# spcl/EBCC

Measured on AMD Instinct MI355X. Metric: fp32 GB/s encode+decode, 721x1440 ERA5 frames MAX_ERROR=0.5, higher is better.
Workload: dtype f32; 1 GPU; 256-frame batch 721x1440 fp32 per GPU, base_cr=30 MAX_ERROR=0.5 (BASELINE configs[1]); frames_per_gpu=256, parallelism=frames sharded over 1 GPU(s), no collective, hw_queues=4, encode_slices=3

## Files before the change

ebcc_amd/csrc/j2k.hip:

```cpp
#include <algorithm>
#include <cstring>
#include <vector>

#include "../../include/ebcc_hip.h"
#include "engine.hpp"
#include "j2k.hpp"

namespace ebcc {

bool j2k_create(ebcc_hip_ctx *ctx)
{
    J2kBuffers *jb = new J2kBuffers();
    ctx->j2k = jb;
    const int period = ctx->tile_period;
    std::vector<std::vector<J2kBlock>> tile_blocks((size_t) period);
    int stride = 0;
    for (int k = 0; k < period; k++) {
        jb->geoms.push_back(make_j2k_geom(ctx->height, ctx->width, tile_blocks[(size_t) k], k * ctx->height));
        stride = std::max(stride, jb->geoms.back().nblocks);
    }
    for (J2kGeom &t : jb->geoms) { t.period = period; t.stride = stride; }
    jb->geom = jb->geoms[0];
    const J2kGeom &g = jb->geom;
    const size_t n_pix = ctx->n_pix, F = ctx->max_frames;
    const size_t total = F * (size_t) stride, groups = (total + 63) / 64;
    jb->max_frames = (int) F;
    jb->fs = ctx->rb.fs;
    jb->stream_cap = ((n_pix * 3 + 4096 + 63) / 64) * 64;
    bool ok = true;
    ok &= (jb->d_geom = (J2kGeom *) ctx_alloc<uint8_t>(ctx, sizeof(J2kGeom) * (size_t) period)) != nullptr;
    ok &= (jb->d_blocks = (J2kBlock *) ctx_alloc<uint8_t>(ctx, sizeof(J2kBlock) * (size_t) period * (size_t) stride)) != nullptr;
    ok &= (jb->d_blkmap = ctx_alloc<uint16_t>(ctx, (size_t) period * n_pix)) != nullptr;
    ok &= (jb->B = ctx_alloc<float>(ctx, F * n_pix)) != nullptr;
    ok &= (jb->B2 = ctx_alloc<float>(ctx, F * n_pix)) != nullptr;
    ok &= (jb->Q6 = ctx_alloc<int32_t>(ctx, F * n_pix)) != nullptr;
    ok &= (jb->DEC = ctx_alloc<float>(ctx, F * n_pix)) != nullptr;
    ok &= (jb->V = ctx_alloc<int32_t>(ctx, F * n_pix)) != nullptr;
    ok &= (jb->BP = ctx_alloc<unsigned long long>(ctx, groups * kJ2kMaxPlanes * 64 * 64)) != nullptr;
    ok &= (jb->SGN = ctx_alloc<unsigned long long>(ctx, groups * 64 * 64)) != nullptr;
    ok &= (jb->SUF = ctx_alloc<unsigned long long>(ctx, groups * (kJ2kMaxPlanes + 2) * 64 * 64)) != nullptr;
    ok &= (jb->SPS = ctx_alloc<unsigned long long>(ctx, groups * 64 * 64)) != nullptr;
    ok &= (jb->VISP = ctx_alloc<unsigned long long>(ctx, groups * kJ2kMaxPlanes * 64 * 64)) != nullptr;
    ok &= (jb->ckpt = ctx_alloc<uint8_t>(ctx, groups * 64 * j2k_ckpt_block_bytes())) != nullptr;
    jb->SYM = nullptr;
    {
        const char *e = getenv("EBCC_T1_TWO_PHASE");
        jb->sym_rows = kJ2kSymRows;
        if (const char *r = getenv("EBCC_HIP_SYM_ROWS")) jb->sym_rows = std::max(1, std::min(kJ2kSymRows, atoi(r)));
        if (!e || atoi(e)) ok &= (jb->SYM = ctx_alloc<uint8_t>(ctx, groups * (size_t) ((jb->sym_rows + 1) & ~1) * 1024 + 256)) != nullptr;
    }
    ok &= (jb->seglen = ctx_alloc<uint16_t>(ctx, groups * (size_t) kJ2kSegCount * 64)) != nullptr;
    ok &= (jb->lanerows = ctx_alloc<uint32_t>(ctx, groups * 64)) != nullptr;
    ok &= (jb->qplane = (int *) ctx_alloc<int32_t>(ctx, groups * 64)) != nullptr;
    ok &= (jb->lastnp = (int *) ctx_alloc<int32_t>(ctx, groups * 64)) != nullptr;
    ok &= (jb->T1S = ctx_alloc<unsigned long long>(ctx, groups * kT1StateWords * 64)) != nullptr;
    ok &= (jb->blkmax = (int *) ctx_alloc<int32_t>(ctx, groups * 64)) != nullptr;
    ok &= (jb->numbps = (int *) ctx_alloc<int32_t>(ctx, groups * 64)) != nullptr;
    ok &= (jb->totalpasses = (int *) ctx_alloc<int32_t>(ctx, groups * 64)) != nullptr;
    ok &= (jb->cblk_len = (int *) ctx_alloc<int32_t>(ctx, groups * 64)) != nullptr;
    ok &= (jb->npass = (int *) ctx_alloc<int32_t>(ctx, groups * 64)) != nullptr;
    ok &= (jb->cand_cr = ctx_alloc<float>(ctx, F * 2)) != nullptr;
    ok &= (jb->cand_out = (int *) ctx_alloc<int32_t>(ctx, F * 6)) != nullptr;
    ok &= (jb->cand_npass = (int *) ctx_alloc<int32_t>(ctx, 2 * F * (size_t) stride)) != nullptr;
    ok &= (jb->cand_sel = (int *) ctx_alloc<int32_t>(ctx, F)) != nullptr;
    ok &= (jb->have_rate = (int *) ctx_alloc<int32_t>(ctx, F)) != nullptr;
    ok &= (jb->rate_path = (int *) ctx_alloc<int32_t>(ctx, F * 1536 * 3)) != nullptr;
    ok &= (jb->rate_path_n = (int *) ctx_alloc<int32_t>(ctx, 2 * F)) != nullptr;
    {
        int nodes = 0;
        for (const J2kGeom &t : jb->geoms) nodes = std::max(nodes, t.tree_nodes);
        J2kBuffers::RateCache &rc = jb->rate_cache;
        rc.nodes_cap = (nodes + 3) & ~3;
        rc.cap = stride * kJ2kMaxPasses;
        rc.ok = jb->rate_path_n ? jb->rate_path_n + F : nullptr;
        ok &= (rc.mnmx = ctx_alloc<double>(ctx, F * 2)) != nullptr;
        ok &= (rc.mval = (short *) ctx_alloc<uint16_t>(ctx, F * (size_t) rc.nodes_cap)) != nullptr;
        ok &= (rc.off = (int *) ctx_alloc<int32_t>(ctx, F * (size_t) (stride + 1))) != nullptr;
        ok &= (rc.crate = ctx_alloc<uint16_t>(ctx, F * (size_t) rc.cap)) != nullptr;
        ok &= (rc.cdisto = ctx_alloc<double>(ctx, F * (size_t) rc.cap)) != nullptr;
    }
    ok &= (jb->rates = (int *) ctx_alloc<int32_t>(ctx, groups * 64 * kJ2kMaxPasses)) != nullptr;
    ok &= (jb->disto = ctx_alloc<double>(ctx, groups * 64 * kJ2kMaxPasses)) != nullptr;
    ok &= (jb->cblk_bytes = ctx_alloc<uint8_t>(ctx, groups * 64 * kJ2kCblkBytes)) != nullptr;
    ok &= (jb->stream = ctx_alloc<uint8_t>(ctx, F * jb->stream_cap)) != nullptr;
    ok &= (jb->dec_table = (int *) ctx_alloc<int32_t>(ctx, groups * 64 * 4)) != nullptr;
    ok &= (jb->dec_order = (int *) ctx_alloc<int32_t>(ctx, groups * 64 + 128)) != nullptr;
    ok &= (jb->mq_order = (int *) ctx_alloc<int32_t>(ctx, groups * 64 + 256)) != nullptr;
    ok &= (jb->jf = (J2kFrame *) ctx_alloc<uint8_t>(ctx, sizeof(J2kFrame) * F)) != nullptr;
    ok &= (jb->partial = ctx_alloc<double>(ctx, F * kPartials)) != nullptr;
    ok &= (jb->partial_u = ctx_alloc<unsigned long long>(ctx, F * kPartials)) != nullptr;
    if (!ok) return false;
    poison_alloc(jb->cblk_bytes, groups * 64 * kJ2kCblkBytes);
    poison_alloc(jb->stream, F * jb->stream_cap);
    if (stride >= 65535) { set_error("too many code-blocks"); return false; }
    std::vector<uint16_t> map((size_t) period * n_pix, 0);
    std::vector<J2kBlock> blocks((size_t) period * (size_t) stride, J2kBlock{});
    for (int k = 0; k < period; k++) {
        const std::vector<J2kBlock> &tb = tile_blocks[(size_t) k];
        std::copy(tb.begin(), tb.end(), blocks.begin() + (size_t) k * (size_t) stride);
        for (size_t b = 0; b < tb.size(); b++)
            for (int y = 0; y < tb[b].h; y++)
                for (int x = 0; x < tb[b].w; x++) map[(size_t) k * n_pix + (size_t) (tb[b].y + y) * g.W + tb[b].x + x] = (uint16_t) b;
    }
    hipStream_t s = ctx->stream;
    EBCC_HIP_CHECK(hipMemcpyAsync(jb->d_geom, jb->geoms.data(), sizeof(J2kGeom) * (size_t) period, hipMemcpyHostToDevice, s));
    EBCC_HIP_CHECK(hipMemcpyAsync(jb->d_blocks, blocks.data(), sizeof(J2kBlock) * blocks.size(), hipMemcpyHostToDevice, s));
    EBCC_HIP_CHECK(hipMemcpyAsync(jb->d_blkmap, map.data(), map.size() * sizeof(uint16_t), hipMemcpyHostToDevice, s));
    EBCC_HIP_CHECK(hipHostMalloc(&ctx->h_jf, sizeof(J2kFrame) * F));
    EBCC_HIP_CHECK(hipHostMalloc((void **) &ctx->h_table, sizeof(int) * 4 * total));
    EBCC_HIP_CHECK(hipMemsetAsync(jb->jf, 0, sizeof(J2kFrame) * F, s));
    EBCC_HIP_CHECK(hipMemsetAsync(jb->rate_path_n, 0, sizeof(int) * 2 * F, s));
    wait_stream(s);
    return true;
}

void j2k_destroy(ebcc_hip_ctx *ctx)
{
    delete static_cast<J2kBuffers *>(ctx->j2k);
    ctx->j2k = nullptr;
    if (ctx->stream2) { hipStreamSynchronize(ctx->stream2); hipStreamDestroy(ctx->stream2); ctx->stream2 = nullptr; }
}

namespace {

struct BitReader {
    const uint8_t *p, *end;
    unsigned buf = 0;
    int ct = 0;
    int bit()
    {
        if (ct == 0) {
            buf = (buf << 8) & 0xFFFF;
            ct = buf == 0xFF00 ? 7 : 8;
            if (p < end) buf |= *p++;
        }
        ct--;
        return (buf >> ct) & 1;
    }
    int bits(int n) { int v = 0; for (int i = n - 1; i >= 0; i--) v |= bit() << i; return v; }
    void align() { if ((buf & 0xFF) == 0xFF && p < end) p++; ct = 0; }
};

struct HostTree {
    const J2kBand *bd;
    std::vector<int> val, low;
    explicit HostTree(const J2kBand &b) : bd(&b)
    {
        int n = 0;
        for (int l = 0; l < b.tree_levels; l++) n += b.lvl_w[l] * b.lvl_h[l];
        val.assign(n, 999); low.assign(n, 0);
    }
    bool decode(BitReader &br, int cx, int cy, int threshold)
    {
        int lowv = 0, idx = 0;
        for (int l = bd->tree_levels - 1; l >= 0; l--) {
            idx = bd->lvl_off[l] + (cy >> l) * bd->lvl_w[l] + (cx >> l);
            if (lowv > low[idx]) low[idx] = lowv; else lowv = low[idx];
            while (lowv < threshold && lowv < val[idx]) {
                if (br.bit()) val[idx] = lowv; else ++lowv;
            }
            low[idx] = lowv;
        }
        return val[idx] < threshold;
    }
// ... 440 lines not shown
```

ebcc_amd/csrc/j2k.hpp:

```cpp
#pragma once

#include <vector>

#include "../../include/ebcc_hip.h"
#include "common.hpp"
#include "residual.hpp"

namespace ebcc {

constexpr int kJ2kRes = 6;
constexpr int kJ2kBands = 3 * kJ2kRes - 2;
constexpr int kJ2kMaxPlanes = 26;
constexpr int kJ2kMaxPasses = 3 * kJ2kMaxPlanes;
constexpr int kJ2kCblkBytes = 16 * 1024;
constexpr int kT1StateWords = 66 + 4 * 64;

struct J2kBand {
    int res, orient, level;
    int x0, y0, x1, y1;
    int offx, offy;
    int ncw, nch;
    int first_block;
    int expn, mant, numbps;
    float step_enc, step_dec;
// ... 35 lines not shown
constexpr int kJ2kSegCount = kJ2kMaxPlanes * 3 * 16;
constexpr int kJ2kSymRows = (4096 * (kJ2kMaxPlanes + 2)) / 16 + kJ2kSegCount;
constexpr int kJ2kCkptPerBlock = kJ2kMaxPasses * 16;

constexpr int kJ2kCkptWords = 8;
__host__ __device__ inline size_t j2k_ckpt_block_bytes() { return (size_t) kJ2kCkptWords * kJ2kCkptPerBlock * 4; }
struct J2kCkptView {
    std::uint32_t *rec;
    __host__ __device__ std::uint32_t *slot(std::uint32_t i) const { return rec + i * kJ2kCkptWords; }
    __host__ __device__ static J2kCkptView of(void *all, size_t gid)
    {
        return J2kCkptView{(std::uint32_t *) ((unsigned char *) all + gid * j2k_ckpt_block_bytes())};
    }
};

struct J2kFrame {
    float cr;
    float target;
    int maxlen;
    int body_bytes;
    int stream_bytes;
    unsigned long long nbad;
    double err_sum;
    int overflow;
    int keep;
    float hdr_share;
    unsigned int bad_limit;
    unsigned int bad_seen;
};

struct J2kBuffers {
    J2kGeom geom;
    std::vector<J2kGeom> geoms;
    J2kGeom *d_geom;
    J2kBlock *d_blocks;
    std::uint16_t *d_blkmap;
    int max_frames;
    float *B;
    float *B2;
    int32_t *Q6;
    float *DEC;
    unsigned long long *BP;
    unsigned long long *SGN;
    unsigned long long *SUF;
    unsigned long long *SPS;
    unsigned long long *VISP;
    void *ckpt;
    uint8_t *SYM;
    int sym_rows;
    std::uint16_t *seglen;
    std::uint32_t *lanerows;
    int *qplane;
    int *lastnp;
    unsigned long long *T1S;
    int *blkmax;
    int *numbps;
    int *totalpasses;
    int *cblk_len;
    int *rates;
    double *disto;
    int *npass;
    float *cand_cr;
    int *cand_out;
    int *cand_npass;
    int *cand_sel;
    int *have_rate;
    int *rate_path;
    int *rate_path_n;
    struct RateCache {
        int *ok;
        double *mnmx;
        short *mval;
        int *off;
        unsigned short *crate;
        double *cdisto;
        int nodes_cap, cap;
    } rate_cache;
    uint8_t *cblk_bytes;
    uint8_t *stream;
    size_t stream_cap;
    int32_t *V;
    int *dec_table;
    int *dec_order;
    int *mq_order;
    J2kFrame *jf;
    FrameState *fs;
    double *partial;
    unsigned long long *partial_u;
};

enum T1Kernel { T1_ENCODE = 0, T1_MQ = 1, T1_RESUME = 2, T1_DECODE = 3 };
int t1_lanes_per_wave(int kernel, int total_blocks = 0);

J2kGeom make_j2k_geom(int H, int W, std::vector<J2kBlock> &blocks, int ty0 = 0);

struct J2kWindow {
    int row0, col0, rows, cols;
    int rx0[kJ2kRes], rx1[kJ2kRes], ry0[kJ2kRes], ry1[kJ2kRes];
    int band[kJ2kBands][4];
};
bool j2k_window_plan(const J2kGeom &g, size_t row0, size_t col0, size_t rows, size_t cols, J2kWindow &w);
bool j2k_window_supported(const J2kGeom &g);
bool j2k_window_keeps(const J2kGeom &g, const J2kBlock &b, const J2kWindow &w, int rect[4]);
constexpr int kL5Pairs = 60;
struct J2kStripRange { int strip0, strips, pos0, pos1, pieces; };
inline J2kStripRange j2k_cone_span(const J2kWindow &w, int r)
{
    const int strip0 = (w.rx0[r] / 2) / kL5Pairs;
    return J2kStripRange{strip0, ((w.rx1[r] - 1) / 2) / kL5Pairs - strip0 + 1, w.ry0[r] / 2, (w.ry1[r] - 1) / 2 + 1, 1};
}
int j2k_first_fused(const J2kBuffers &jb);
struct J2kBoxEntry {
    int frame, slot, row0, col0;
    int strip0[kJ2kRes], strips[kJ2kRes], pos0[kJ2kRes], pos1[kJ2kRes];
    int pad[4];
};
struct J2kPlacement {
    int rows, cols;
    unsigned long long at, pitch;
};
struct J2kBoxList {
    J2kBoxEntry *h_table, *table;
    J2kPlacement *h_place, *place;
    size_t n;
    int rows, cols;
};
struct J2kRegion {
    enum Kind { Frames, Window, List } kind = Frames;
    J2kWindow cone{};
    J2kBoxList list{};
    float *out = nullptr;
};
bool j2k_list_check(const char *who, const J2kGeom &g, size_t n_frames, const ebcc_hip_placed_box *boxes, size_t n_boxes, size_t out_floats,
                    uint8_t *keep = nullptr, J2kBoxEntry *table = nullptr, J2kPlacement *place = nullptr, int first_fused = kJ2kRes,
                    int *max_rows = nullptr, int *max_cols = nullptr);
bool j2k_boxes_as_placed(const char *who, const ebcc_hip_box *boxes, size_t n_boxes, size_t rows, size_t cols,
                         std::vector<ebcc_hip_placed_box> &placed, size_t *out_floats);
int j2k_selfcheck_div65535();

void launch_input_stats(const float *data, int n_frames, size_t n_pix, FrameState *fs, hipStream_t s);
void launch_j2k_analysis(const float *data, const J2kBuffers &jb, int n_frames, hipStream_t s);
void launch_j2k_tier1(const J2kBuffers &jb, int n_frames, hipStream_t s, bool single_kernel);
bool j2k_tier1_retry(const J2kBuffers &jb, int n_frames, const J2kFrame *host_jf, hipStream_t s);
// ... 14 lines not shown
```

ebcc_amd/csrc/j2k_rate.hip:

```cpp
#include <cfloat>
#include <cmath>
#include <cstdlib>
#include <mutex>

#include "j2k.hpp"
#include "t1_core.hpp"
#include "t1_device.hpp"

namespace ebcc {

int j2k_inverse_dwt(float *B, const int32_t *V, const float *data, const J2kBuffers &jb, int n_frames, const FrameState *fs,
                    const int *active, hipStream_t s, int keep_field, const J2kWindow *win = nullptr, float *win_out = nullptr);

namespace {

constexpr int kMainHeaderBytes = 135;
constexpr int kRateTrieNodes = 1536;
#ifndef EBCC_RATE_THREADS
#define EBCC_RATE_THREADS 512
#endif
constexpr int kRateThreads = EBCC_RATE_THREADS;
constexpr int kWriteThreads = 256;

__device__ inline int floorlog2d(int a) { return a > 1 ? 31 - __clz(a) : 0; }
// ... 876 lines not shown
        int running = 0;
        for (int base_b = 0; base_b < g.nblocks; base_b += kWriteThreads) {
            const int b = base_b + lane;
            int v = 0;
            if (b < g.nblocks && L.npass[b]) v = rates[(size_t) (gid0 + b) * kJ2kMaxPasses + L.npass[b] - 1];
            int x = v;
            for (int d = 1; d < 64; d <<= 1) { const int y = __shfl_up(x, d); if ((lane & 63) >= d) x += y; }
            if ((lane & 63) == 63) s_wave[lane >> 6] = x;
            __syncthreads();
            int before = running, tot = 0;
            for (int w = 0; w < kWriteThreads / 64; w++) { if (w < (lane >> 6)) before += s_wave[w]; tot += s_wave[w]; }
            if (b < g.nblocks) L.leafbits[b] = before + x - v;
            running += tot;
            __syncthreads();
        }
    }
    {
        const int wave = lane >> 6, wl = lane & 63;
        for (int blk = wave; blk < g.nblocks; blk += kWriteThreads / 64) {
            const int n = L.npass[blk];
            if (!n) continue;
            int bi = 0;
            while (bi + 1 < g.nbands && g.bands[bi + 1].first_block <= blk) bi++;
            const int res = g.bands[bi].res;
            const int seglen = rates[(size_t) (gid0 + blk) * kJ2kMaxPasses + n - 1];
            const uint8_t *src = cblk_bytes + (size_t) (gid0 + blk) * kJ2kCblkBytes;
            uint8_t *dst = base + s_off[res] + s_hdr[res] + (L.leafbits[blk] - L.leafbits[g.res_first[res]]);
            for (int i = wl; i < seglen; i += 64) dst[i] = src[i];
        }
    }
    if (lane == 0) {
        uint8_t *p = base;
        put16(p, 0xFF4F);
        put16(p, 0xFF51); put16(p, 41); put16(p, 0);
        put32(p, g.W); put32(p, g.H); put32(p, 0); put32(p, 0); put32(p, g.W); put32(p, g.H); put32(p, 0); put32(p, 0);
        put16(p, 1); *p++ = 15; *p++ = 1; *p++ = 1;
        put16(p, 0xFF52); put16(p, 12); *p++ = 0; *p++ = 0; put16(p, 1); *p++ = 0; *p++ = kJ2kRes - 1; *p++ = 4; *p++ = 4; *p++ = 0; *p++ = 0;
        put16(p, 0xFF5C); put16(p, 3 + 2 * kJ2kBands); *p++ = (uint8_t) (2 + (2 << 5));
        for (int bi = 0; bi < kJ2kBands; bi++) put16(p, (unsigned) ((g.bands[bi].expn << 11) | g.bands[bi].mant));
        const char com[] = "Created by OpenJPEG version 2.4.0";
        put16(p, 0xFF64); put16(p, 4 + 33); put16(p, 1);
        for (int i = 0; i < 33; i++) *p++ = (uint8_t) com[i];
        const int body = s_off[kJ2kRes] - (kMainHeaderBytes + 14);
        put16(p, 0xFF90); put16(p, 10); put16(p, 0); put32(p, (unsigned) (12 + 2 + body)); *p++ = 0; *p++ = 1;
        put16(p, 0xFF93);
        uint8_t *e = base + s_off[kJ2kRes];
        put16(e, 0xFFD9);
        jf[frame].stream_bytes = s_off[kJ2kRes] + 2;
        jf[frame].body_bytes = body;
    }
}

__global__ void k_finish_reduce(const double *partial, const unsigned long long *partial_u, J2kFrame *jf, int n, int n_partials,
                                const FrameState *fs, const int *active)
{
    int f = blockIdx.x * blockDim.x + threadIdx.x;
    if (f >= n || (active && !active[f]) || fs[f].const_field) return;
    jf[f].bad_seen = 0;
    double s = 0;
    unsigned long long b = 0;
    for (int i = 0; i < n_partials; i++) { s += partial[(size_t) f * kPartials + i]; b += partial_u[(size_t) f * kPartials + i]; }
    jf[f].err_sum = s;
    jf[f].nbad = b;
}


struct LdsTable {
    const __attribute__((address_space(3))) uint32_t *t;
    __device__ uint32_t operator()(int i) const { return t[i]; }
};
#define EBCC_LDS_MQ_TABLE(name)                                                              \
    __shared__ uint32_t name##_store[48];                                                    \
    if (threadIdx.x < 47) name##_store[threadIdx.x] = t1::mq_entry((int) threadIdx.x);       \
    __syncthreads();                                                                         \
    LdsTable name{(const __attribute__((address_space(3))) uint32_t *) name##_store}

__device__ __attribute__((aligned(16))) uint8_t g_ctx_tables[LdsCtx::kBytes];
void ensure_ctx_tables()
{
    static std::once_flag once[64];
    int dev = 0;
    EBCC_HIP_CHECK(hipGetDevice(&dev));
    std::call_once(once[dev & 63], [] {
        uint8_t t[LdsCtx::kBytes];
        make_ctx_tables(t);
        EBCC_HIP_CHECK(hipMemcpyToSymbol(HIP_SYMBOL(g_ctx_tables), t, sizeof t));
    });
}

struct DecStore {
    unsigned char *st;
    uint32_t lane8;
    int32_t *v;
    int W;
    __device__ unsigned long long &at(int row) const { return *(unsigned long long *) (st + ((uint32_t) row * 512u + lane8)); }
    __device__ unsigned long long &S(int y) { return at(y + 1); }
    __device__ unsigned long long &NEG(int y) { return at(66 + y); }
    __device__ unsigned long long &VIS(int y) { return at(130 + y); }
    __device__ unsigned long long &REF(int y) { return at(194 + y); }
    __device__ void set_sig(int x, int y, int neg, int plane)
    {
        int one = 1 << (plane + 1), val = one | (one >> 1);
        v[y * W + x] = neg ? -val : val;
    }
    __device__ void refine(int x, int y, int bit, int plane, int neg)
    {
        const int half = 1 << plane;
        atomicAdd(&v[y * W + x], (bit ^ neg) ? half : -half);
    }
// ... 147 lines not shown
    EBCC_LDS_MQ_TABLE(tab);
    const LdsCtx ctxp{(uint32_t) (uintptr_t) (__attribute__((address_space(3))) uint8_t *) ctx_store, 0u};
    int w = (int) blockIdx.x, slot0 = 0, lanes = tiers.lanes[3], end = total;
    {
        int t = 0;
        for (; t < 3; t++) {
            const int waves = tiers.n[t] / tiers.lanes[t];
            if (w < waves) { lanes = tiers.lanes[t]; end = slot0 + tiers.n[t]; break; }
            w -= waves; slot0 += tiers.n[t];
        }
    }
    if ((int) threadIdx.x >= lanes) return;
    const int slot = slot0 + w * lanes + (int) threadIdx.x;
    if (slot >= end || slot >= total) return;
    const int gid = order[slot];
    const int nb = geom->stride;
    const int frame = gid / nb, bi = gid - frame * nb;
    if (fs[frame].const_field) return;
    blocks = j2k_frame_blocks(geom, blocks, frame);
    geom = &j2k_frame_geom(geom, frame);
    const int *e = dec_table + (size_t) gid * 4;
    const int len = e[1], P = e[2], np = e[3];
    const uint8_t *src = bytes + (size_t) frame * stream_cap + e[0];
    if (np <= 0 || P <= 0) return;
    const J2kBlock blk = blocks[bi];
    DecStoreLds st{(uint32_t) (uintptr_t) (__attribute__((address_space(3))) unsigned long long *) dec_state + threadIdx.x * 8u, (uint32_t) lanes * 8u,
                   V + (size_t) frame * geom->W * geom->H + (size_t) blk.y * geom->W + blk.x, geom->W};
    for (int r = 0; r < kDecStateRows; r++) st.at(r) = 0ull;
    t1::decode_block(st, DecSrcSeq(src, len), blk.w, blk.h, geom->bands[blk.band].orient, P, np, tab, ctxp);
}


constexpr int kProbeHistRounds = 96, kProbeHistFrames = 4096;
__device__ unsigned int g_probe_hist[kProbeHistRounds][8];
__device__ unsigned int g_probe_round;
__device__ int g_probe_minres[kProbeHistFrames];
__device__ unsigned int g_probe_fine_changed[kProbeHistFrames];
__device__ unsigned int g_probe_tiles[kProbeHistFrames][4];
__device__ unsigned long long g_probe_dirty[kProbeHistRounds];
__global__ void k_probe_hist_round(int n_frames, const FrameState *fs, const int *active)
{
    const int f = blockIdx.x * blockDim.x + threadIdx.x;
    const unsigned int round = min(g_probe_round, (unsigned int) kProbeHistRounds - 1);
    if (f < n_frames && f < kProbeHistFrames && !((active && !active[f]) || fs[f].const_field)) {
        const int m = g_probe_minres[f];
        atomicAdd(&g_probe_hist[round][m > 5 ? 6 : m], 1u);
        if (m == 5) atomicAdd(&g_probe_hist[round][7], g_probe_fine_changed[f]);
        atomicAdd(&g_probe_dirty[round], (unsigned long long) (__popc(g_probe_tiles[f][0]) + __popc(g_probe_tiles[f][1]) + __popc(g_probe_tiles[f][2])));
    }
    if (f < kProbeHistFrames) { g_probe_minres[f] = 99; g_probe_fine_changed[f] = 0; g_probe_tiles[f][0] = g_probe_tiles[f][1] = g_probe_tiles[f][2] = 0; }
}
__global__ void k_probe_hist_next() { g_probe_round++; }

__global__ void k_probe_plan(const int *__restrict__ numbps, const int *__restrict__ npass, const int *__restrict__ rates,
                             void *ckpt, int *__restrict__ rpass, int *__restrict__ lastnp, const J2kGeom *geom,
                             const J2kBlock *blocks, const FrameState *fs, const int *active, int total, int stats)
{
    const int gid = blockIdx.x * blockDim.x + threadIdx.x;
    if (gid >= total) return;
    const int frame = gid / geom->stride;
    if ((active && !active[frame]) || fs[frame].const_field) return;
    const int n = npass[gid], P = numbps[gid];
    if (lastnp[gid] == n) { rpass[gid] = -2; return; }
    if (stats && frame < kProbeHistFrames && lastnp[gid] != -1) {
        const int res = j2k_frame_geom(geom, frame).bands[j2k_frame_blocks(geom, blocks, frame)[gid - frame * geom->stride].band].res;
        atomicMin(&g_probe_minres[frame], res);
        if (res == 5) atomicAdd(&g_probe_fine_changed[frame], 1u);
        const J2kGeom &g = j2k_frame_geom(geom, frame);
        const J2kBlock &b = j2k_frame_blocks(geom, blocks, frame)[gid - frame * geom->stride];
        const J2kBand &bd = g.bands[b.band];
        const int sc = 1 << (res == 0 ? 5 : 6 - res), bx = b.x - bd.offx, by = b.y - bd.offy;
        const int x0 = max(0, (bx - 5) * sc), x1 = min(g.W - 1, (bx + b.w + 5) * sc), y0 = max(0, (by - 5) * sc), y1 = min(g.H - 1, (by + b.h + 5) * sc);
        const int th = (g.H + 7) / 8;
        for (int ty = y0 / th; ty <= y1 / th; ty++)
            for (int tx = x0 / 120; tx <= x1 / 120; tx++) { const int t = ty * 12 + tx; if (t < 96) atomicOr(&g_probe_tiles[frame][t >> 5], 1u << (t & 31)); }
    }
    lastnp[gid] = n;
    int plan = -1;
    if (n > 0 && P > 0) {
        const int len = rates[(size_t) gid * kJ2kMaxPasses + n - 1];
        const int nstr = (j2k_frame_blocks(geom, blocks, frame)[gid - frame * geom->stride].h + 3) >> 2;
        const J2kCkptView ck = J2kCkptView::of(ckpt, (size_t) gid);
        int lo = 0, hi = n * nstr - 1;
        while (lo < hi) {
            const int mid = (lo + hi + 1) >> 1;
            const int mp = mid / nstr, ms = mid - mp * nstr;
            if ((int) ck.slot((uint32_t) (mp * 16 + ms))[1] + 1 < len) lo = mid; else hi = mid - 1;
        }
        const int r = lo / nstr, st = lo - r * nstr;
        plan = r | (st << 8);
    }
    rpass[gid] = plan;
}

__global__ __launch_bounds__(256) void k_probe_init(const int32_t *__restrict__ Q6, const int *__restrict__ rpass,
                                                     const int *__restrict__ numbps, const unsigned long long *__restrict__ SPS,
                                                     int32_t *__restrict__ V, const J2kGeom *geom, const J2kBlock *blocks,
                                                     const FrameState *fs, const int *active)
{
    const int frame = blockIdx.y, bi = blockIdx.x;
    if ((active && !active[frame]) || fs[frame].const_field) return;
    const int gid = frame * geom->stride + bi;
    const int plan = rpass[gid];
    if (plan == -2) return;
    if (bi >= j2k_frame_geom(geom, frame).nblocks) return;
    const int W = geom->W;
    const size_t n_pix = (size_t) W * geom->H;
    const J2kBlock blk = j2k_frame_blocks(geom, blocks, frame)[bi];
    const int P = numbps[gid];
    const int x = threadIdx.x & 63;
    if (x >= blk.w) return;
    const int32_t *q = Q6 + (size_t) frame * n_pix + (size_t) blk.y * W + blk.x + x;
    int32_t *v = V + (size_t) frame * n_pix + (size_t) blk.y * W + blk.x + x;
    const unsigned long long *spsrow = SPS + ((size_t) (gid >> 6) * 64) * 64 + (gid & 63);
    for (int y = threadIdx.x >> 6; y < blk.h; y += 4) {
        const int q6 = q[(size_t) y * W];
        const unsigned int a = (unsigned int) (q6 < 0 ? -q6 : q6) >> 6;
        int out = 0;
        if (plan > 0 && a) {
            const int bs = 31 - __clz(a);
            const int r = (plan & 0xFF) + (y < 4 * (plan >> 8) ? 1 : 0);
            const unsigned long long sps = spsrow[(size_t) y * 64];
            const int ps = bs == P - 1 ? 0 : 3 * (P - 1 - bs) - (((sps >> x) & 1ull) ? 2 : 0);
            if (ps < r) {
                out = 3 << bs;
                for (int pl = bs - 1; pl >= 0; pl--) {
                    if (3 * (P - 1 - pl) - 1 >= r) break;
                    out += ((a >> pl) & 1u) ? (1 << pl) : -(1 << pl);
                }
                if (q6 < 0) out = -out;
            }
        }
        v[(size_t) y * W] = out;
    }
}

__global__ __launch_bounds__(64) void k_t1_resume(unsigned long long *T1S, const unsigned long long *BP,
                                                   const unsigned long long *SUF, const unsigned long long *SGN,
                                                   const unsigned long long *SPS, const unsigned long long *VISP,
                                                   const uint8_t *cblk_bytes, const int *numbps, const int *npass,
                                                   const int *rates, const int *rpass, void *ckpt, int32_t *V,
                                                   const J2kGeom *geom, const J2kBlock *blocks, const FrameState *fs,
                                                   const int *active, int total, int lpw)
{
    extern __shared__ unsigned long long dec_state[];
    __shared__ __attribute__((aligned(16))) uint8_t ctx_store[LdsCtx::kBytes];
    EBCC_LDS_MQ_TABLE(tab);
    const int gid0 = blockIdx.x * lpw;
    const int gid = gid0 + threadIdx.x;
    const int nb = geom->stride;
    int plan = -1, frame = 0, bi = 0;
    if ((int) threadIdx.x < lpw && gid < total) {
        frame = gid / nb; bi = gid - frame * nb;
        if (!((active && !active[frame]) || fs[frame].const_field)) plan = rpass[gid];
    }
    if (!__any(plan >= 0)) return;
    copy_ctx_tables(ctx_store, g_ctx_tables, (int) threadIdx.x, 64);
    __syncthreads();
    if (plan < 0) return;
    const LdsCtx ctxp{(uint32_t) (uintptr_t) (__attribute__((address_space(3))) uint8_t *) ctx_store, 0u};
    blocks = j2k_frame_blocks(geom, blocks, frame);
    geom = &j2k_frame_geom(geom, frame);
    const int r = plan & 0xFF, stripe = plan >> 8;
    const int np = npass[gid], P = numbps[gid];
    const int len = rates[(size_t) gid * kJ2kMaxPasses + np - 1];
    const J2kBlock blk = blocks[bi];
    const size_t grp = (size_t) (gid0 >> 6);
    const int gl = (gid0 & 63) + threadIdx.x;
    DecStoreLds st{(uint32_t) (uintptr_t) (__attribute__((address_space(3))) unsigned long long *) dec_state + threadIdx.x * 8u, (uint32_t) lpw * 8u,
                   V + (size_t) frame * geom->W * geom->H + (size_t) blk.y * geom->W + blk.x, geom->W};
    const unsigned long long *sg = SGN + grp * 64 * 64 + gl;
    const unsigned long long *sps = SPS + grp * 64 * 64 + gl;
    st.S(-1) = 0; st.S(64) = 0;
    const int y_first = r == np - 1 ? max(0, 4 * stripe - 1) & ~3 : 0;
    for (int y0 = y_first; y0 < 64; y0 += 4) {
        unsigned long long s1[4], s2[4], bpv[4], spv[4], vv[4], sgv[4];
        int tt[4];
#pragma unroll
        for (int k = 0; k < 4; k++) {
            const int y = y0 + k;
            const int q = r + (y < 4 * stripe ? 1 : 0);
            tt[k] = -1; s1[k] = s2[k] = bpv[k] = spv[k] = vv[k] = sgv[k] = 0ull;
            if (y < blk.h && q > 0) {
                const int p = t1::plane_of_pass(P, q), t = t1::type_of_pass(q);
                tt[k] = t;
                s1[k] = SUF[((grp * (kJ2kMaxPlanes + 2) + p + 1) * 64 + y) * 64 + gl];
                if (t >= 1) {
                    spv[k] = sps[(size_t) y * 64];
                    bpv[k] = BP[((grp * kJ2kMaxPlanes + p) * 64 + y) * 64 + gl];
                    vv[k] = VISP[((grp * kJ2kMaxPlanes + p) * 64 + y) * 64 + gl];
                }
                if (t != 2) s2[k] = SUF[((grp * (kJ2kMaxPlanes + 2) + p + 2) * 64 + y) * 64 + gl];
                sgv[k] = sg[(size_t) y * 64];
            }
        }
#pragma unroll
        for (int k = 0; k < 4; k++) {
            const int y = y0 + k;
            unsigned long long S = 0, R = 0, Vv = 0;
            if (tt[k] >= 0) {
                S = s1[k];
                if (tt[k] >= 1) { S |= spv[k] & bpv[k] & ~s1[k]; Vv = vv[k]; }
                R = tt[k] == 2 ? s1[k] : s2[k];
            }
            st.S(y) = S;
            st.NEG(y) = sgv[k] & S;
            st.REF(y) = R;
            st.VIS(y) = Vv;
        }
    }
    const J2kCkptView cv = J2kCkptView::of(ckpt, (size_t) gid);
    const uint4 *rec = (const uint4 *) cv.slot((uint32_t) (r * 16 + stripe));
    const uint4 r0 = rec[0], r1 = rec[1];
    const uint32_t cxb[5] = {r0.z, r0.w, r1.x, r1.y, r1.z};
    const t1::Contexts cxp = t1::Contexts::from_bytes(cxb);
    const t1::MqCheckpoint ck{r0.x & 0xFFFFu, r1.w, (int) (r0.x >> 16), (int) r0.y, cxp.w0, cxp.w1, cxp.w2};
    t1::decode_resume(st, DecSrc{cblk_bytes + (size_t) gid * kJ2kCblkBytes, len}, blk.w, blk.h, geom->bands[blk.band].orient, P,
                      np, r, stripe, ck, tab, ctxp);
}

size_t rate_lds(const J2kBuffers &jb)
{
    size_t n = 0;
    for (const J2kGeom &g : jb.geoms) n = std::max(n, rate_lds_bytes(g.nblocks, g.tree_nodes));
    return n;
}

}

static void rate_launch(const J2kBuffers &jb, int n_frames, const int *d_active, hipStream_t s, bool candidates, const int *have_rate)
{
    const size_t head = ((rate_lds(jb) + 15) & ~(size_t) 15) + rate_off_bytes(jb.geom.stride) + rate_path_bytes(jb.geom.stride);
    const size_t budget = 150 * 1024;
    size_t want = (size_t) jb.geom.stride * kJ2kMaxPasses;
    if (head + want * 10 + 16 > budget) want = head + 16 < budget ? (budget - head - 16) / 10 : 0;
    const size_t lds = head + want * 10 + 16;
    static std::once_flag once;
    std::call_once(once, [] {
        EBCC_HIP_CHECK(hipFuncSetAttribute((const void *) k_rate, hipFuncAttributeMaxDynamicSharedMemorySize, 150 * 1024));
    });
    hipLaunchKernelGGL(k_rate, dim3(n_frames, candidates ? 2 : 1), dim3(kRateThreads), lds, s, jb.numbps, jb.totalpasses, jb.rates,
                       jb.disto, candidates ? jb.cand_npass : jb.npass, jb.d_geom, jb.jf, jb.fs, d_active, (int) want, jb.rate_path, jb.rate_path_n,
                       candidates ? jb.cand_cr : nullptr, jb.cand_out, (size_t) jb.max_frames * (size_t) jb.geom.stride, have_rate, jb.rate_cache);
    EBCC_HIP_LAUNCH_CHECK();
}

void launch_j2k_rate(const J2kBuffers &jb, int n_frames, const int *d_active, hipStream_t s, const int *have_rate)
{
    ScopedTiming t("rate_alloc", s);
    rate_launch(jb, n_frames, d_active, s, false, have_rate);
}

void launch_j2k_rate_candidates(const J2kBuffers &jb, int n_frames, const int *d_active, hipStream_t s)
{
    rate_launch(jb, n_frames, d_active, s, true, nullptr);
}

__global__ void k_rate_publish(const int *sel, const int *cand_npass, const int *cand_out, size_t cand_stride, int *npass, J2kFrame *jf,
                               const J2kGeom *geom, int *have_rate)
{
    const int frame = blockIdx.x, c = sel[frame];
    if (threadIdx.x == 0) have_rate[frame] = c >= 0 ? 1 : 0;
    if (c < 0) return;
    const int nb = geom->stride;
    const int *src = cand_npass + (size_t) c * cand_stride + (size_t) frame * nb;
    for (int b = threadIdx.x; b < nb; b += blockDim.x) npass[(size_t) frame * nb + b] = src[b];
    if (threadIdx.x == 0) {
        const int *o = cand_out + (size_t) (2 * frame + c) * 3;
        jf[frame].body_bytes = o[0]; jf[frame].stream_bytes = o[1]; jf[frame].maxlen = o[2];
    }
}
void launch_j2k_rate_publish(const J2kBuffers &jb, int n_frames, hipStream_t s)
{
    hipLaunchKernelGGL(k_rate_publish, dim3(n_frames), dim3(64), 0, s, jb.cand_sel, jb.cand_npass, jb.cand_out,
                       (size_t) jb.max_frames * (size_t) jb.geom.stride, jb.npass, jb.jf, jb.d_geom, jb.have_rate);
    EBCC_HIP_LAUNCH_CHECK();
}

void launch_j2k_write(const J2kBuffers &jb, int n_frames, const int *d_active, hipStream_t s)
{
    hipLaunchKernelGGL(k_write, dim3(n_frames), dim3(kWriteThreads), rate_lds(jb), s, jb.numbps, jb.rates, jb.npass,
                       jb.cblk_bytes, jb.stream, jb.stream_cap, jb.d_geom, jb.jf, jb.fs, d_active);
    EBCC_HIP_LAUNCH_CHECK();
}

static void decode_tail(const float *data, const J2kBuffers &jb, int n_frames, const int *d_active, bool stats, hipStream_t s,
                        int keep_field = 1, const J2kWindow *win = nullptr, float *win_out = nullptr)
{
    const int partials = j2k_inverse_dwt(jb.B, jb.V, stats ? data : nullptr, jb, n_frames, jb.fs, d_active, s, keep_field, win, win_out);
    if (stats)
        hipLaunchKernelGGL(k_finish_reduce, dim3(ceil_div(n_frames, 64)), dim3(64), 0, s, jb.partial, jb.partial_u, jb.jf,
                           n_frames, partials, jb.fs, d_active);
}

void launch_j2k_probe_decode(const float *data, const J2kBuffers &jb, int n_frames, const int *d_active, hipStream_t s, int keep_field)
{
    const int total = n_frames * jb.geom.stride;
    void *ck = jb.ckpt;
    static const bool stats = getenv("EBCC_HIP_T1_STATS") != nullptr;
    hipLaunchKernelGGL(k_probe_plan, dim3(ceil_div(total, 256)), dim3(256), 0, s, jb.numbps, jb.npass, jb.rates, ck, jb.qplane,
                       jb.lastnp, jb.d_geom, jb.d_blocks, jb.fs, d_active, total, stats ? 1 : 0);
    if (stats) {
        hipLaunchKernelGGL(k_probe_hist_round, dim3(ceil_div(std::max(n_frames, kProbeHistFrames), 256)), dim3(256), 0, s, n_frames, jb.fs, d_active);
        hipLaunchKernelGGL(k_probe_hist_next, dim3(1), dim3(1), 0, s);
    }
    hipLaunchKernelGGL(k_probe_init, dim3(jb.geom.stride, n_frames), dim3(256), 0, s, jb.Q6, jb.qplane, jb.numbps, jb.SPS, jb.V,
                       jb.d_geom, jb.d_blocks, jb.fs, d_active);
    timing_begin("t1_probe_decode", s);
    const int lpw = t1_lanes_per_wave(T1_RESUME);
    ensure_ctx_tables();
    hipLaunchKernelGGL(k_t1_resume, dim3((unsigned) ceil_div(total, lpw)), dim3(64), (size_t) kDecStateRows * lpw * 8, s, jb.T1S, jb.BP, jb.SUF, jb.SGN, jb.SPS,
                       jb.VISP, jb.cblk_bytes, jb.numbps, jb.npass, jb.rates, jb.qplane, ck, jb.V, jb.d_geom, jb.d_blocks, jb.fs,
                       d_active, total, lpw);
    timing_end("t1_probe_decode", s);
    decode_tail(data, jb, n_frames, d_active, true, s, keep_field);
    EBCC_HIP_LAUNCH_CHECK();
    EBCC_HIP_LAUNCH_CHECK();
}

void j2k_probe_hist_dump(const char *what)
{
    unsigned int h[kProbeHistRounds][8], rounds = 0, zero = 0;
    unsigned long long dirty[kProbeHistRounds];
    EBCC_HIP_CHECK(hipMemcpyFromSymbol(h, HIP_SYMBOL(g_probe_hist), sizeof h));
    EBCC_HIP_CHECK(hipMemcpyFromSymbol(dirty, HIP_SYMBOL(g_probe_dirty), sizeof dirty));
    EBCC_HIP_CHECK(hipMemcpyFromSymbol(&rounds, HIP_SYMBOL(g_probe_round), sizeof rounds));
    fprintf(stderr, "ebcc-mi355x probes of %s, per round: frames by the coarsest resolution with a changed code-block [0 1 2 3 4 5 none] (changed finest code-blocks per frame of class 5)\n", what);
    for (unsigned int r = 0; r < std::min(rounds, (unsigned int) kProbeHistRounds); r++) {
        unsigned int n = 0;
        for (int k = 0; k < 7; k++) n += h[r][k];
        if (!n) continue;
        fprintf(stderr, "ebcc-mi355x   round %2u: %4u %4u %4u %4u %4u %4u %4u  (%.1f)  tiles reached %.1f %%\n", r, h[r][0], h[r][1], h[r][2], h[r][3], h[r][4], h[r][5], h[r][6],
                h[r][5] ? (double) h[r][7] / h[r][5] : 0.0, 100.0 * (double) dirty[r] / (96.0 * n));
    }
    static unsigned long long zd[kProbeHistRounds];
    EBCC_HIP_CHECK(hipMemcpyToSymbol(HIP_SYMBOL(g_probe_dirty), zd, sizeof zd));
    static unsigned int zeros[kProbeHistRounds][8];
    EBCC_HIP_CHECK(hipMemcpyToSymbol(HIP_SYMBOL(g_probe_hist), zeros, sizeof zeros));
    EBCC_HIP_CHECK(hipMemcpyToSymbol(HIP_SYMBOL(g_probe_round), &zero, sizeof zero));
}

constexpr double kDecChainMsPerByte = 3.0e-3;
constexpr double kDecIssueMsPerByte[3] = {1.0e-6, 0.82e-6, 0.706e-6};
static DecTiers plan_dec_tiers(const int *host_table, int total)
{
    long long cnt[kDecClasses] = {0};
    double all = 0;
    int longest = 0;
    for (int i = 0; i < total; i++) {
        const int *e = host_table + (size_t) i * 4;
        const int c = e[3] <= 0 || e[2] <= 0 ? 0 : std::min(kDecClasses - 1, 1 + (e[1] >> 6));
        cnt[c]++;
        if (c) { all += e[1]; longest = std::max(longest, e[1]); }
    }
    int c64 = kDecClasses - 1;
    for (long long above = 0; c64 > 0 && above + cnt[c64] <= total / kDecTierDen1; c64--) above += cnt[c64];
    const double len64 = std::min((double) longest, 64.0 * c64);
    const double alone = std::max(kDecChainMsPerByte * longest, kDecIssueMsPerByte[0] * all);
    const double pairs = std::max(2 * 0.875 * kDecChainMsPerByte * longest, kDecIssueMsPerByte[1] * all);
    const double fours = std::max({2 * 0.875 * kDecChainMsPerByte * longest, 4 * 0.68 * kDecChainMsPerByte * len64, kDecIssueMsPerByte[2] * all});
    DecTiers tiers{{0, 0, 0}, {1, 2, 4, 4}};
    if (alone <= pairs && alone <= fours) tiers.lanes[3] = 1;
    else if (pairs <= fours) tiers.lanes[3] = 2;
    else tiers.n[1] = total / kDecTierDen1 / 2 * 2;
    return tiers;
}
// ... 88 lines not shown
```

Measured before the change: 8.931 GB/s.

## Compact changed code-blocks into a worklist and fuse probe init into resume

The probe planning kernel now builds a compacted list of code-blocks whose pass count changed, using wave ballot and an atomic counter. A new list-driven resume kernel spreads only those blocks over the grid, fuses the per-block probe initialisation (batched row loads) into the same kernel, and then runs the T1 resume decode. This avoids launching the separate init kernel and scanning every block, at the cost of atomics, an extra count reset in finish_reduce, and a grid still sized for all blocks. Correctness depends on unchanged blocks keeping their V values from earlier probes, which the old init kernel handled by writing zeros or values for every block.

```diff
diff --git a/ebcc_amd/csrc/j2k.hip b/ebcc_amd/csrc/j2k.hip
--- a/ebcc_amd/csrc/j2k.hip
+++ b/ebcc_amd/csrc/j2k.hip
@@ -52,7 +52,8 @@
     ok &= (jb->seglen = ctx_alloc<uint16_t>(ctx, groups * (size_t) kJ2kSegCount * 64)) != nullptr;
     ok &= (jb->lanerows = ctx_alloc<uint32_t>(ctx, groups * 64)) != nullptr;
     ok &= (jb->qplane = (int *) ctx_alloc<int32_t>(ctx, groups * 64)) != nullptr;
-    ok &= (jb->lastnp = (int *) ctx_alloc<int32_t>(ctx, groups * 64)) != nullptr;
+    ok &= (jb->lastnp = (int *) ctx_alloc<int32_t>(ctx, groups * 64 * 2 + 1)) != nullptr;
+    jb->changed = jb->lastnp ? jb->lastnp + groups * 64 : nullptr;
     ok &= (jb->T1S = ctx_alloc<unsigned long long>(ctx, groups * kT1StateWords * 64)) != nullptr;
     ok &= (jb->blkmax = (int *) ctx_alloc<int32_t>(ctx, groups * 64)) != nullptr;
     ok &= (jb->numbps = (int *) ctx_alloc<int32_t>(ctx, groups * 64)) != nullptr;
@@ -110,6 +111,7 @@
     EBCC_HIP_CHECK(hipHostMalloc((void **) &ctx->h_table, sizeof(int) * 4 * total));
     EBCC_HIP_CHECK(hipMemsetAsync(jb->jf, 0, sizeof(J2kFrame) * F, s));
     EBCC_HIP_CHECK(hipMemsetAsync(jb->rate_path_n, 0, sizeof(int) * 2 * F, s));
+    EBCC_HIP_CHECK(hipMemsetAsync(jb->changed, 0, sizeof(int) * (groups * 64 + 1), s));
     wait_stream(s);
     return true;
 }
diff --git a/ebcc_amd/csrc/j2k.hpp b/ebcc_amd/csrc/j2k.hpp
--- a/ebcc_amd/csrc/j2k.hpp
+++ b/ebcc_amd/csrc/j2k.hpp
@@ -111,6 +111,7 @@
     std::uint32_t *lanerows;
     int *qplane;
     int *lastnp;
+    int *changed;
     unsigned long long *T1S;
     int *blkmax;
     int *numbps;
@@ -148,6 +149,8 @@
     unsigned long long *partial_u;
 };
 
+inline int j2k_changed_cap(const J2kBuffers &jb) { return jb.max_frames * jb.geom.stride; }
+
 enum T1Kernel { T1_ENCODE = 0, T1_MQ = 1, T1_RESUME = 2, T1_DECODE = 3 };
 int t1_lanes_per_wave(int kernel, int total_blocks = 0);
 
diff --git a/ebcc_amd/csrc/j2k_rate.hip b/ebcc_amd/csrc/j2k_rate.hip
--- a/ebcc_amd/csrc/j2k_rate.hip
+++ b/ebcc_amd/csrc/j2k_rate.hip
@@ -952,9 +952,10 @@
 }
 
 __global__ void k_finish_reduce(const double *partial, const unsigned long long *partial_u, J2kFrame *jf, int n, int n_partials,
-                                const FrameState *fs, const int *active)
+                                const FrameState *fs, const int *active, int *list_count)
 {
     int f = blockIdx.x * blockDim.x + threadIdx.x;
+    if (f == 0 && list_count) *list_count = 0;
     if (f >= n || (active && !active[f]) || fs[f].const_field) return;
     jf[f].bad_seen = 0;
     double s = 0;
@@ -1208,16 +1209,14 @@
 }
 __global__ void k_probe_hist_next() { g_probe_round++; }
 
-__global__ void k_probe_plan(const int *__restrict__ numbps, const int *__restrict__ npass, const int *__restrict__ rates,
-                             void *ckpt, int *__restrict__ rpass, int *__restrict__ lastnp, const J2kGeom *geom,
-                             const J2kBlock *blocks, const FrameState *fs, const int *active, int total, int stats)
-{
-    const int gid = blockIdx.x * blockDim.x + threadIdx.x;
-    if (gid >= total) return;
+__device__ int probe_plan_block(int gid, const int *__restrict__ numbps, const int *__restrict__ npass, const int *__restrict__ rates,
+                                void *ckpt, int *__restrict__ rpass, int *__restrict__ lastnp, const J2kGeom *geom,
+                                const J2kBlock *blocks, const FrameState *fs, const int *active, int stats)
+{
     const int frame = gid / geom->stride;
-    if ((active && !active[frame]) || fs[frame].const_field) return;
+    if ((active && !active[frame]) || fs[frame].const_field) return -3;
     const int n = npass[gid], P = numbps[gid];
-    if (lastnp[gid] == n) { rpass[gid] = -2; return; }
+    if (lastnp[gid] == n) { rpass[gid] = -2; return -2; }
     if (stats && frame < kProbeHistFrames && lastnp[gid] != -1) {
         const int res = j2k_frame_geom(geom, frame).bands[j2k_frame_blocks(geom, blocks, frame)[gid - frame * geom->stride].band].res;
         atomicMin(&g_probe_minres[frame], res);
@@ -1247,6 +1246,53 @@
         plan = r | (st << 8);
     }
     rpass[gid] = plan;
+    return plan;
+}
+
+__global__ void k_probe_plan(const int *__restrict__ numbps, const int *__restrict__ npass, const int *__restrict__ rates,
+                             void *ckpt, int *__restrict__ rpass, int *__restrict__ lastnp, const J2kGeom *geom,
+                             const J2kBlock *blocks, const FrameState *fs, const int *active, int total, int stats,
+                             int *__restrict__ list, int *count, int cap)
+{
+    const int gid = blockIdx.x * blockDim.x + threadIdx.x;
+    int plan = -3;
+    if (gid < total) plan = probe_plan_block(gid, numbps, npass, rates, ckpt, rpass, lastnp, geom, blocks, fs, active, stats);
+    if (!list) return;
+    bool listed = false;
+    if (plan >= -1) {
+        const int frame = gid / geom->stride;
+        listed = gid - frame * geom->stride < j2k_frame_geom(geom, frame).nblocks;
+    }
+    const unsigned long long m = __ballot(listed);
+    if (!m) return;
+    const int lane = (int) (threadIdx.x & 63u), first = __ffsll((long long) m) - 1;
+    int base = 0;
+    if (lane == first) base = atomicAdd(count, __popcll(m));
+    base = __shfl(base, first);
+    const int at = base + __popcll(m & ((1ull << lane) - 1ull));
+    if (listed && at < cap) list[at] = gid;
+}
+
+template <class Sps>
+__device__ __forceinline__ int probe_init_value(int q6, int plan, int x, int y, int P, Sps sps_of_row)
+{
+    const unsigned int a = (unsigned int) (q6 < 0 ? -q6 : q6) >> 6;
+    int out = 0;
+    if (plan > 0 && a) {
+        const int bs = 31 - __clz(a);
+        const int r = (plan & 0xFF) + (y < 4 * (plan >> 8) ? 1 : 0);
+        const unsigned long long sps = sps_of_row();
+        const int ps = bs == P - 1 ? 0 : 3 * (P - 1 - bs) - (((sps >> x) & 1ull) ? 2 : 0);
+        if (ps < r) {
+            out = 3 << bs;
+            for (int pl = bs - 1; pl >= 0; pl--) {
+                if (3 * (P - 1 - pl) - 1 >= r) break;
+                out += ((a >> pl) & 1u) ? (1 << pl) : -(1 << pl);
+            }
+            if (q6 < 0) out = -out;
+        }
+    }
+    return out;
 }
 
 __global__ __launch_bounds__(256) void k_probe_init(const int32_t *__restrict__ Q6, const int *__restrict__ rpass,
@@ -1269,62 +1315,28 @@
     const int32_t *q = Q6 + (size_t) frame * n_pix + (size_t) blk.y * W + blk.x + x;
     int32_t *v = V + (size_t) frame * n_pix + (size_t) blk.y * W + blk.x + x;
     const unsigned long long *spsrow = SPS + ((size_t) (gid >> 6) * 64) * 64 + (gid & 63);
-    for (int y = threadIdx.x >> 6; y < blk.h; y += 4) {
-        const int q6 = q[(size_t) y * W];
-        const unsigned int a = (unsigned int) (q6 < 0 ? -q6 : q6) >> 6;
-        int out = 0;
-        if (plan > 0 && a) {
-            const int bs = 31 - __clz(a);
-            const int r = (plan & 0xFF) + (y < 4 * (plan >> 8) ? 1 : 0);
-            const unsigned long long sps = spsrow[(size_t) y * 64];
-            const int ps = bs == P - 1 ? 0 : 3 * (P - 1 - bs) - (((sps >> x) & 1ull) ? 2 : 0);
-            if (ps < r) {
-                out = 3 << bs;
-                for (int pl = bs - 1; pl >= 0; pl--) {
-                    if (3 * (P - 1 - pl) - 1 >= r) break;
-                    out += ((a >> pl) & 1u) ? (1 << pl) : -(1 << pl);
-                }
-                if (q6 < 0) out = -out;
-            }
-        }
-        v[(size_t) y * W] = out;
-    }
-}
-
-__global__ __launch_bounds__(64) void k_t1_resume(unsigned long long *T1S, const unsigned long long *BP,
-                                                   const unsigned long long *SUF, const unsigned long long *SGN,
-                                                   const unsigned long long *SPS, const unsigned long long *VISP,
-                                                   const uint8_t *cblk_bytes, const int *numbps, const int *npass,
-                                                   const int *rates, const int *rpass, void *ckpt, int32_t *V,
-                                                   const J2kGeom *geom, const J2kBlock *blocks, const FrameState *fs,
-                                                   const int *active, int total, int lpw)
-{
-    extern __shared__ unsigned long long dec_state[];
-    __shared__ __attribute__((aligned(16))) uint8_t ctx_store[LdsCtx::kBytes];
-    EBCC_LDS_MQ_TABLE(tab);
-    const int gid0 = blockIdx.x * lpw;
-    const int gid = gid0 + threadIdx.x;
+    for (int y = threadIdx.x >> 6; y < blk.h; y += 4)
+        v[(size_t) y * W] = probe_init_value(q[(size_t) y * W], plan, x, y, P, [&] { return spsrow[(size_t) y * 64]; });
+}
+
+__device__ __forceinline__ void t1_resume_block(int gid, int plan, uint32_t lds_base, uint32_t lds_stride, const unsigned long long *BP,
+                                                const unsigned long long *SUF, const unsigned long long *SGN,
+                                                const unsigned long long *SPS, const unsigned long long *VISP,
+                                                const uint8_t *cblk_bytes, const int *numbps, const int *npass, const int *rates,
+                                                void *ckpt, int32_t *V, const J2kGeom *geom, const J2kBlock *blocks,
+                                                const LdsTable &tab, const LdsCtx &ctxp)
+{
     const int nb = geom->stride;
-    int plan = -1, frame = 0, bi = 0;
-    if ((int) threadIdx.x < lpw && gid < total) {
-        frame = gid / nb; bi = gid - frame * nb;
-        if (!((active && !active[frame]) || fs[frame].const_field)) plan = rpass[gid];
-    }
-    if (!__any(plan >= 0)) return;
-    copy_ctx_tables(ctx_store, g_ctx_tables, (int) threadIdx.x, 64);
-    __syncthreads();
-    if (plan < 0) return;
-    const LdsCtx ctxp{(uint32_t) (uintptr_t) (__attribute__((address_space(3))) uint8_t *) ctx_store, 0u};
+    const int frame = gid / nb, bi = gid - frame * nb;
     blocks = j2k_frame_blocks(geom, blocks, frame);
     geom = &j2k_frame_geom(geom, frame);
     const int r = plan & 0xFF, stripe = plan >> 8;
     const int np = npass[gid], P = numbps[gid];
     const int len = rates[(size_t) gid * kJ2kMaxPasses + np - 1];
     const J2kBlock blk = blocks[bi];
-    const size_t grp = (size_t) (gid0 >> 6);
-    const int gl = (gid0 & 63) + threadIdx.x;
-    DecStoreLds st{(uint32_t) (uintptr_t) (__attribute__((address_space(3))) unsigned long long *) dec_state + threadIdx.x * 8u, (uint32_t) lpw * 8u,
-                   V + (size_t) frame * geom->W * geom->H + (size_t) blk.y * geom->W + blk.x, geom->W};
+    const size_t grp = (size_t) (gid >> 6);
+    const int gl = gid & 63;
+    DecStoreLds st{lds_base, lds_stride, V + (size_t) frame * geom->W * geom->H + (size_t) blk.y * geom->W + blk.x, geom->W};
     const unsigned long long *sg = SGN + grp * 64 * 64 + gl;
     const unsigned long long *sps = SPS + grp * 64 * 64 + gl;
     st.S(-1) = 0; st.S(64) = 0;
@@ -1375,6 +1387,91 @@
                       np, r, stripe, ck, tab, ctxp);
 }
 
+__global__ __launch_bounds__(64) void k_t1_resume(unsigned long long *T1S, const unsigned long long *BP,
+                                                   const unsigned long long *SUF, const unsigned long long *SGN,
+                                                   const unsigned long long *SPS, const unsigned long long *VISP,
+                                                   const uint8_t *cblk_bytes, const int *numbps, const int *npass,
+                                                   const int *rates, const int *rpass, void *ckpt, int32_t *V,
+                                                   const J2kGeom *geom, const J2kBlock *blocks, const FrameState *fs,
+                                                   const int *active, int total, int lpw)
+{
+    extern __shared__ unsigned long long dec_state[];
+    __shared__ __attribute__((aligned(16))) uint8_t ctx_store[LdsCtx::kBytes];
+    EBCC_LDS_MQ_TABLE(tab);
+    const int gid0 = blockIdx.x * lpw;
+    const int gid = gid0 + threadIdx.x;
+    int plan = -1;
+    if ((int) threadIdx.x < lpw && gid < total) {
+        const int frame = gid / geom->stride;
+        if (!((active && !active[frame]) || fs[frame].const_field)) plan = rpass[gid];
+    }
+    if (!__any(plan >= 0)) return;
+    copy_ctx_tables(ctx_store, g_ctx_tables, (int) threadIdx.x, 64);
+    __syncthreads();
+    if (plan < 0) return;
+    const LdsCtx ctxp{(uint32_t) (uintptr_t) (__attribute__((address_space(3))) uint8_t *) ctx_store, 0u};
+    t1_resume_block(gid, plan, (uint32_t) (uintptr_t) (__attribute__((address_space(3))) unsigned long long *) dec_state + threadIdx.x * 8u,
+                    (uint32_t) lpw * 8u, BP, SUF, SGN, SPS, VISP, cblk_bytes, numbps, npass, rates, ckpt, V, geom, blocks, tab, ctxp);
+}
+
+__global__ __launch_bounds__(64) void k_t1_resume_list(const int *__restrict__ list, const int *__restrict__ count, int cap,
+                                                        const int32_t *__restrict__ Q6, const unsigned long long *BP,
+                                                        const unsigned long long *SUF, const unsigned long long *SGN,
+                                                        const unsigned long long *SPS, const unsigned long long *VISP,
+                                                        const uint8_t *cblk_bytes, const int *numbps, const int *npass,
+                                                        const int *rates, const int *rpass, void *ckpt, int32_t *V,
+                                                        const J2kGeom *geom, const J2kBlock *blocks, int lpw)
+{
+    extern __shared__ unsigned long long dec_state[];
+    __shared__ __attribute__((aligned(16))) uint8_t ctx_store[LdsCtx::kBytes];
+    const int n_list = min(*count, cap);
+    const int per = min(lpw, (n_list + (int) gridDim.x - 1) / (int) gridDim.x);
+    const int e0 = blockIdx.x * per;
+    if (e0 >= n_list) return;
+    EBCC_LDS_MQ_TABLE(tab);
+    const int mine = min(per, n_list - e0);
+    const int nb = geom->stride, W = geom->W;
+    const size_t n_pix = (size_t) W * geom->H;
+    for (int e = 0; e < mine; e++) {
+        const int gid = __builtin_amdgcn_readfirstlane(list[e0 + e]);
+        const int plan = rpass[gid];
+        if (plan < -1) continue;
+        const int frame = gid / nb;
+        const J2kBlock blk = j2k_frame_blocks(geom, blocks, frame)[gid - frame * nb];
+        const int x = (int) threadIdx.x;
+        if (x >= blk.w) continue;
+        const int P = numbps[gid];
+        const int32_t *q = Q6 + (size_t) frame * n_pix + (size_t) blk.y * W + blk.x + x;
+        int32_t *v = V + (size_t) frame * n_pix + (size_t) blk.y * W + blk.x + x;
+        const unsigned long long *spsrow = SPS + ((size_t) (gid >> 6) * 64) * 64 + (gid & 63);
+        for (int y0 = 0; y0 < blk.h; y0 += 16) {
+            int q6[16];
+            unsigned long long sps[16];
+#pragma unroll
+            for (int k = 0; k < 16; k++) {
+                const int y = min(y0 + k, blk.h - 1);
+                q6[k] = q[(size_t) y * W];
+                sps[k] = spsrow[(size_t) y * 64];
+            }
+#pragma unroll
+            for (int k = 0; k < 16; k++) {
+                const int y = y0 + k;
+                if (y < blk.h) v[(size_t) y * W] = probe_init_value(q6[k], plan, x, y, P, [&] { return sps[k]; });
+            }
+        }
+    }
+    __threadfence_block();
+    int plan = -1, gid = 0;
+    if ((int) threadIdx.x < mine) { gid = list[e0 + threadIdx.x]; plan = rpass[gid]; }
+    if (!__any(plan >= 0)) return;
+    copy_ctx_tables(ctx_store, g_ctx_tables, (int) threadIdx.x, 64);
+    __syncthreads();
+    if (plan < 0) return;
+    const LdsCtx ctxp{(uint32_t) (uintptr_t) (__attribute__((address_space(3))) uint8_t *) ctx_store, 0u};
+    t1_resume_block(gid, plan, (uint32_t) (uintptr_t) (__attribute__((address_space(3))) unsigned long long *) dec_state + threadIdx.x * 8u,
+                    (uint32_t) lpw * 8u, BP, SUF, SGN, SPS, VISP, cblk_bytes, numbps, npass, rates, ckpt, V, geom, blocks, tab, ctxp);
+}
+
 size_t rate_lds(const J2kBuffers &jb)
 {
     size_t n = 0;
@@ -1446,7 +1543,13 @@
     const int partials = j2k_inverse_dwt(jb.B, jb.V, stats ? data : nullptr, jb, n_frames, jb.fs, d_active, s, keep_field, win, win_out);
     if (stats)
         hipLaunchKernelGGL(k_finish_reduce, dim3(ceil_div(n_frames, 64)), dim3(64), 0, s, jb.partial, jb.partial_u, jb.jf,
-                           n_frames, partials, jb.fs, d_active);
+                           n_frames, partials, jb.fs, d_active, jb.changed + j2k_changed_cap(jb));
+}
+
+static bool probe_list_enabled()
+{
+    const char *e = getenv("EBCC_HIP_PROBE_LIST");
+    return !e || atoi(e) != 0;
 }
 
 void launch_j2k_probe_decode(const float *data, const J2kBuffers &jb, int n_frames, const int *d_active, hipStream_t s, int keep_field)
@@ -1454,20 +1557,29 @@
     const int total = n_frames * jb.geom.stride;
     void *ck = jb.ckpt;
     static const bool stats = getenv("EBCC_HIP_T1_STATS") != nullptr;
+    const bool by_list = probe_list_enabled();
+    const int cap = j2k_changed_cap(jb);
     hipLaunchKernelGGL(k_probe_plan, dim3(ceil_div(total, 256)), dim3(256), 0, s, jb.numbps, jb.npass, jb.rates, ck, jb.qplane,
-                       jb.lastnp, jb.d_geom, jb.d_blocks, jb.fs, d_active, total, stats ? 1 : 0);
+                       jb.lastnp, jb.d_geom, jb.d_blocks, jb.fs, d_active, total, stats ? 1 : 0, by_list ? jb.changed : nullptr,
+                       jb.changed + cap, cap);
     if (stats) {
         hipLaunchKernelGGL(k_probe_hist_round, dim3(ceil_div(std::max(n_frames, kProbeHistFrames), 256)), dim3(256), 0, s, n_frames, jb.fs, d_active);
         hipLaunchKernelGGL(k_probe_hist_next, dim3(1), dim3(1), 0, s);
     }
-    hipLaunchKernelGGL(k_probe_init, dim3(jb.geom.stride, n_frames), dim3(256), 0, s, jb.Q6, jb.qplane, jb.numbps, jb.SPS, jb.V,
-                       jb.d_geom, jb.d_blocks, jb.fs, d_active);
+    if (!by_list)
+        hipLaunchKernelGGL(k_probe_init, dim3(jb.geom.stride, n_frames), dim3(256), 0, s, jb.Q6, jb.qplane, jb.numbps, jb.SPS, jb.V,
+                           jb.d_geom, jb.d_blocks, jb.fs, d_active);
     timing_begin("t1_probe_decode", s);
     const int lpw = t1_lanes_per_wave(T1_RESUME);
     ensure_ctx_tables();
-    hipLaunchKernelGGL(k_t1_resume, dim3((unsigned) ceil_div(total, lpw)), dim3(64), (size_t) kDecStateRows * lpw * 8, s, jb.T1S, jb.BP, jb.SUF, jb.SGN, jb.SPS,
-                       jb.VISP, jb.cblk_bytes, jb.numbps, jb.npass, jb.rates, jb.qplane, ck, jb.V, jb.d_geom, jb.d_blocks, jb.fs,
-                       d_active, total, lpw);
+    if (by_list)
+        hipLaunchKernelGGL(k_t1_resume_list, dim3((unsigned) ceil_div(total, lpw)), dim3(64), (size_t) kDecStateRows * lpw * 8, s, jb.changed,
+                           jb.changed + cap, cap, jb.Q6, jb.BP, jb.SUF, jb.SGN, jb.SPS, jb.VISP, jb.cblk_bytes, jb.numbps, jb.npass, jb.rates,
+                           jb.qplane, ck, jb.V, jb.d_geom, jb.d_blocks, lpw);
+    else
+        hipLaunchKernelGGL(k_t1_resume, dim3((unsigned) ceil_div(total, lpw)), dim3(64), (size_t) kDecStateRows * lpw * 8, s, jb.T1S, jb.BP, jb.SUF, jb.SGN, jb.SPS,
+                           jb.VISP, jb.cblk_bytes, jb.numbps, jb.npass, jb.rates, jb.qplane, ck, jb.V, jb.d_geom, jb.d_blocks, jb.fs,
+                           d_active, total, lpw);
     timing_end("t1_probe_decode", s);
     decode_tail(data, jb, n_frames, d_active, true, s, keep_field);
     EBCC_HIP_LAUNCH_CHECK();
```

Measured after the change: 9.002 GB/s, median of 6. About the same (+0.8%).
